# qianyizh/ElasticReconstruction

Measured on AMD Instinct MI355X. Metric: depth frames/sec into 512^3 TSDF (640x480), higher is better.
Workload: dtype f32; 1 GPU; configs[1]; frames_per_gpu=91800, volume_units_touched=122, warp=True, inputs=hbm_resident, parallelism=single GPU

## Files before the change

### elasticreconstruction_amd/_ffi.py

```python
import ctypes as C
import os

_HERE = os.path.dirname(os.path.abspath(__file__))
LIB_PATH = os.environ.get("ER_HIP_LIB") or os.path.join(_HERE, "liber_hip.so")

SYMBOLS = [
    "er_last_error", "er_device_count", "er_abi_version", "er_request_hw_queues", "er_host_alloc", "er_host_free", "er_host_copy_h2d", "er_device_alloc", "er_device_free", "er_device_copy_d2h",
    "er_tsdf_create", "er_tsdf_destroy", "er_tsdf_set_stream", "er_tsdf_synchronize",
    "er_tsdf_wait_event", "er_tsdf_reset", "er_tsdf_status", "er_tsdf_set_unit_shard", "er_unit_owner",
    "er_tsdf_scale_depth", "er_tsdf_reproject", "er_tsdf_integrate", "er_tsdf_integrate_frames",
    "er_tsdf_unit_count", "er_tsdf_unit_keys", "er_tsdf_read_unit", "er_tsdf_sum_weight",
    "er_tsdf_extract_world", "er_tsdf_extract_surface", "er_tsdf_extract_oriented", "er_tsdf_extract_mesh", "er_mc_table", "er_tsdf_extract_mesh_indexed", "er_tsdf_import_world", "er_raycast_params_default", "er_tsdf_raycast", "er_tsdf_raycast_batch", "er_tsdf_export_weighted", "er_tsdf_import_weighted",
    "er_tsdf_export_raw", "er_tsdf_import_raw",
    "er_tsdf_color_enable", "er_tsdf_read_unit_color", "er_tsdf_write_unit_color", "er_tsdf_color_frames", "er_tsdf_reproject_color", "er_tsdf_sample_colors",
    "er_tsdf_band_sizes", "er_tsdf_export_band", "er_tsdf_merge_band", "er_tsdf_import_band", "er_tsdf_drop_units",
    "er_tsdf_set_profiling", "er_tsdf_get_profile",
    "er_comm_unique_id", "er_comm_create", "er_comm_create_local", "er_comm_create_loopback", "er_comm_destroy", "er_comm_rank", "er_comm_world",
    "er_tsdf_allreduce", "er_comm_merge_stats", "er_comm_merge_stats_owner", "er_frame_block",
    "er_cloud_create", "er_cloud_create_batch", "er_cloud_create_from_tsdf", "er_cloud_destroy", "er_cloud_size",
    "er_icp_count_inliers", "er_icp_align", "er_icp_align_trace", "er_find_correspondence",
    "er_icp_count_inliers_batch", "er_icp_align_batch", "er_find_correspondence_batch", "er_icp_release_workspaces", "er_registration_batch", "er_ransac_fitness_batch", "er_ransac_inliers",
    "er_features_create", "er_features_destroy", "er_features_size", "er_feature_knn", "er_ransac_hypotheses", "er_ransac_params_default", "er_ransac_align", "er_ransac_align_batch",
    "er_odom_params_default", "er_odom_create", "er_odom_destroy", "er_odom_align_pairs", "er_odom_track", "er_frame_to_model_align", "er_frames_to_models_align", "er_odom_linearize", "er_odom_read_maps", "er_odom_tables",
    "er_cloud_read", "er_cloud_voxel_grid", "er_cloud_estimate_normals", "er_fpfh_estimate", "er_features_dim", "er_features_read",
    "er_frag_params_default", "er_frag_create", "er_frag_destroy", "er_frag_lane_bytes", "er_frag_build", "er_frag_count", "er_frag_read",
    "er_pgo_create", "er_pgo_destroy", "er_pgo_optimize", "er_pgo_set_state", "er_pgo_get_state", "er_pgo_linearize", "er_pgo_trial", "er_pgo_set_profiling", "er_pgo_get_profile",
    "er_fopt_create", "er_fopt_destroy", "er_fopt_set_cloud", "er_fopt_cloud_size", "er_fopt_get_points", "er_fopt_update_pose",
    "er_fopt_update_point_pn", "er_fopt_set_correspondences", "er_fopt_set_correspondences_dev", "er_fopt_group_count", "er_fopt_group_info", "er_fopt_update_normals", "er_fopt_assemble_rigid", "er_fopt_assemble_slac",
    "er_fopt_assemble_nonrigid", "er_fopt_factor_slac", "er_fopt_factor_nonrigid", "er_fopt_solve", "er_fopt_debug_shift_diagonal",
]


class ErWarp(C.Structure):
    _fields_ = [
        ("ctr", C.POINTER(C.c_float)),
        ("num_grids", C.c_int),
        ("resolution", C.c_int),
        ("length", C.c_float),
        ("grid_index", C.POINTER(C.c_int)),
        ("seg", C.POINTER(C.c_double)),
        ("madj", C.POINTER(C.c_double)),
    ]

# ... 34 lines not shown
        return _lib
    if not os.path.exists(LIB_PATH):
        raise ErError(
            "liber_hip.so not found at %s -- build it with `python -c 'import __graft_entry__ as g; g.build()'` "
            "or `make -C elasticreconstruction_amd/csrc`; there is no CPU fallback." % LIB_PATH)
    L = C.CDLL(LIB_PATH, mode=C.RTLD_GLOBAL)
    vp, ip, dp, fp = C.c_void_p, C.POINTER(C.c_int), C.POINTER(C.c_double), C.POINTER(C.c_float)
    u16p = C.POINTER(C.c_uint16)
    L.er_last_error.restype = C.c_char_p
    L.er_last_error.argtypes = []
    L.er_device_count.argtypes = []
    L.er_abi_version.argtypes = []
    L.er_host_alloc.restype = vp
    L.er_host_alloc.argtypes = [C.c_size_t]
    L.er_host_free.argtypes = [vp]
    L.er_host_copy_h2d.argtypes = [vp, vp, C.c_size_t]
    L.er_device_alloc.restype = vp
    L.er_device_alloc.argtypes = [C.c_size_t, C.c_int]
    L.er_device_free.argtypes = [vp]
    L.er_device_copy_d2h.argtypes = [vp, vp, C.c_size_t]
    L.er_tsdf_create.argtypes = [C.c_int, C.c_int, fp, C.c_int, C.c_int, C.POINTER(vp)]
    L.er_tsdf_destroy.argtypes = [vp]
    L.er_tsdf_set_stream.argtypes = [vp, vp]
    L.er_tsdf_synchronize.argtypes = [vp]
    L.er_tsdf_wait_event.argtypes = [vp, vp]
    L.er_tsdf_reset.argtypes = [vp]
    L.er_tsdf_status.argtypes = [vp, ip, C.POINTER(C.c_long)]
    L.er_tsdf_set_unit_shard.argtypes = [vp, C.c_int, C.c_int]
    L.er_unit_owner.argtypes = [C.c_int, C.c_int]
    L.er_tsdf_scale_depth.argtypes = [vp, vp, vp]
    L.er_tsdf_reproject.argtypes = [vp, vp, vp, C.c_int, C.c_float, vp, vp]
    L.er_tsdf_integrate.argtypes = [vp, vp, vp]
    L.er_tsdf_integrate_frames.argtypes = [vp, C.c_int, vp, C.c_int, vp, C.POINTER(ErWarp)]
    L.er_tsdf_unit_count.argtypes = [vp, ip]
    L.er_tsdf_unit_keys.argtypes = [vp, vp]
    L.er_tsdf_read_unit.argtypes = [vp, C.c_int, vp, vp]
    L.er_tsdf_sum_weight.argtypes = [vp, dp]
    L.er_tsdf_extract_world.argtypes = [vp, vp, C.c_long, C.POINTER(C.c_long)]
    L.er_tsdf_extract_surface.argtypes = [vp, vp, C.c_long, C.POINTER(C.c_long)]
    if hasattr(L, "er_tsdf_extract_oriented"):
        L.er_tsdf_extract_oriented.argtypes = [vp, vp, vp, C.c_long, C.POINTER(C.c_long)]
    L.er_tsdf_extract_mesh.argtypes = [vp, vp, C.c_long, C.POINTER(C.c_long)]
    L.er_mc_table.argtypes = [vp]
    if hasattr(L, "er_tsdf_extract_mesh_indexed"):
        L.er_tsdf_extract_mesh_indexed.argtypes = [vp, vp, vp, C.c_long, vp, C.c_long, C.POINTER(C.c_long), C.POINTER(C.c_long)]
        L.er_tsdf_import_world.argtypes = [vp, vp, C.c_long, ip]
    if hasattr(L, "er_tsdf_raycast"):
        L.er_raycast_params_default.argtypes = [C.POINTER(ErRaycastParams)]
        L.er_tsdf_raycast.argtypes = [vp, C.c_int, C.c_int, vp, vp, C.POINTER(ErRaycastParams), vp, vp, C.c_int]
    if hasattr(L, "er_tsdf_raycast_batch"):
        L.er_tsdf_raycast_batch.argtypes = [C.c_int, vp, vp, vp, vp, vp, vp, vp, vp]
    if hasattr(L, "er_frag_create"):
        L.er_frag_params_default.argtypes = [C.POINTER(ErFragParams)]
        L.er_frag_create.argtypes = [C.c_int, C.c_int, vp, C.POINTER(ErOdomParams), C.POINTER(ErFragParams), C.c_int, C.POINTER(vp)]
        L.er_frag_destroy.argtypes = [vp]
        L.er_frag_lane_bytes.argtypes = [vp, C.POINTER(C.c_size_t)]
        L.er_frag_build.argtypes = [vp, C.c_int, vp, C.c_int, vp, C.c_int, vp, vp]
        L.er_frag_count.argtypes = [vp, ip]
        L.er_frag_read.argtypes = [vp, C.c_int, vp, vp, C.c_long, C.POINTER(C.c_long)]
    if hasattr(L, "er_tsdf_color_enable"):
        L.er_tsdf_color_enable.argtypes = [vp]
        L.er_tsdf_read_unit_color.argtypes = [vp, C.c_int, vp]
        L.er_tsdf_write_unit_color.argtypes = [vp, C.c_int, vp]
        L.er_tsdf_color_frames.argtypes = [vp, C.c_int, vp, vp, C.c_int, vp, C.POINTER(ErWarp), vp]
        L.er_tsdf_sample_colors.argtypes = [vp, vp, C.c_long, vp, vp]
        L.er_tsdf_reproject_color.argtypes = [vp, vp, vp, vp, C.c_int, C.c_float, vp, vp]
# ... 158 lines not shown
```

### elasticreconstruction_amd/csrc/er_tsdf.h

```cpp
#pragma once

#include "er_common.h"
#include "er_tsdf_math.h"

#include "../../include/er_hip.h"

#include <algorithm>
#include <cstdlib>
#include <utility>
#include <vector>

namespace er_tsdf_k {
using namespace er;

constexpr int kBlock = 256;
constexpr int kEmptyKey = -1;
constexpr uint32_t kZEmpty = 0xFFFFFFFFu;

enum { C_NUNITS = 0, C_NBATCH = 1 , C_POOL_OVERFLOW = 2, C_TABLE_FULL = 3, C_OUT_OF_RANGE = 4,
       C_NBATCH1 = 6, C_NBATCH2 = 7, C_ZERO_WRITE = 8 ,
       C_ZERO_WRITE1 = 10, C_COUNT = 12 };
constexpr int kDepth = 3;
constexpr int kAux = 2;

struct ReprojArgs {
  const uint16_t* depth;
  int n_frames, cols, rows;
  Camera cam;
  CameraInv cami;
  const double* seg12;
  const double* madj12;
  const int* grid_index;
  const float* ctr;
  int res;
  float grid_ul;
  int floats_per_grid;
  uint32_t* zbuf;
  uint32_t* lastzero;
  uint32_t* zfix;
  int* zero_flag;
};
__global__ void k_reproject_scatter(ReprojArgs A);

constexpr int kFixThreads = 64;
constexpr int kFixBlocks = 256;

constexpr int kScaledPad = 64;
constexpr int kTile = 32;
constexpr int kLoShift = 4;
constexpr int kLoSub = kTile >> kLoShift;
constexpr int kTileKeys = 96;

constexpr int kPrepThreads = 256;
constexpr int kPrepPix = kTile * kTile / kPrepThreads;

__global__ __launch_bounds__(kPrepThreads) void k_prepare(
    const uint16_t* __restrict__ depth, uint32_t* __restrict__ zbuf, int n_frames, int cols, int rows,
    Camera cam, CameraInv cami, const float* __restrict__ lambda, const double* __restrict__ T12, float* __restrict__ scaled,
    int* __restrict__ ht_key, int* __restrict__ ht_slot, unsigned long long* __restrict__ ht_mask, int cap_mask,
    int hash_shift, int* __restrict__ batch, int* __restrict__ nbatch,
    int* __restrict__ counters, float* __restrict__ tile_max, float* __restrict__ tile_lo, float* __restrict__ tile_lo_fine, int2 shard,
    uint32_t* __restrict__ lastzero, uint32_t* __restrict__ zfix, const int* __restrict__ zero_flag);

constexpr int kRows = 4;
constexpr int kItemsPerUnit = 256;

struct Plan {
  int n_units;
  int next;
};

struct PlanRec {
  int key;
  int slot;
  unsigned long long mask;
};

constexpr int kIntMinBlocks = 5;

template <bool kSure>
__global__ __launch_bounds__(kBlock, kIntMinBlocks) void k_integrate(
    float2* __restrict__ pool, const PlanRec* __restrict__ plan_rec, Plan* __restrict__ plan,
    const FrameXform* __restrict__ frames, const float* __restrict__ scaled, const float* __restrict__ tile_max,
    const float* __restrict__ tile_lo, const float* __restrict__ tile_lo_fine, int tiles_x, int tiles_y, Camera cam, int cols, int rows);
extern template __global__ void k_integrate<true>(float2* __restrict__, const PlanRec* __restrict__, Plan* __restrict__, const FrameXform* __restrict__, const float* __restrict__, const float* __restrict__, const float* __restrict__, const float* __restrict__, int, int, Camera, int, int);
extern template __global__ void k_integrate<false>(float2* __restrict__, const PlanRec* __restrict__, Plan* __restrict__, const FrameXform* __restrict__, const float* __restrict__, const float* __restrict__, const float* __restrict__, const float* __restrict__, int, int, Camera, int, int);
}

struct er_tsdf_s {
  int device = 0, cols = 0, rows = 0, pixels = 0, max_units = 0;
  er::Camera cam{};
  er::CameraInv cami{};
  hipStream_t own_stream = nullptr, stream = nullptr;
  hipEvent_t caller_ev = nullptr;
  hipEvent_t voxel_done = nullptr;
// ... 57 lines not shown
```

### elasticreconstruction_amd/csrc/er_tsdf.hip

```cpp
#include "er_tsdf_dev.h"

namespace {

using namespace er_tsdf_k;

constexpr int kNbatchSlot[3] = {C_NBATCH, C_NBATCH1, C_NBATCH2};
constexpr int kZeroFlagSlot[2] = {C_ZERO_WRITE, C_ZERO_WRITE1};

__global__ void k_lambda(float* __restrict__ lambda, int cols, int rows, Camera cam) {
  int p = blockIdx.x * blockDim.x + threadIdx.x;
  if (p >= cols * rows) return;
  lambda[p] = scale_lambda(p % cols, p / cols, cam);
}

__global__ void k_scale_depth(const uint16_t* __restrict__ depth, const float* __restrict__ lambda,
                              float* __restrict__ scaled, int pixels, float itrunc) {
  int p = blockIdx.x * blockDim.x + threadIdx.x;
  if (p >= pixels) return;
  scaled[p] = scale_depth_px(depth[p], lambda[p], itrunc);
}

__global__ __launch_bounds__(kFixThreads) __attribute__((amdgpu_num_vgpr(48))) void k_reproject_fix(ReprojArgs A) {
  const int fl0 = A.zero_flag[0], fl1 = A.zero_flag[1];
  if ((fl0 | fl1) == 0) return;
// ... 296 lines not shown
  const double* dev_seg = reinterpret_cast<const double*>(dst + offsetof(Staging, seg));
  const double* dev_madj = reinterpret_cast<const double*>(dst + offsetof(Staging, madj));
  const int* dev_gi = reinterpret_cast<const int*>(dst + offsetof(Staging, gi));
  if (warp) {
    for (int f = 0; f < n; f++) {
      for (int q = 0; q < 12; q++) {
        st->seg[f * 16 + q] = warp->seg[(size_t)(frame0 + f) * 16 + q];
        st->madj[f * 12 + q] = warp->madj[(size_t)(frame0 + f) * 16 + q];
      }
      er::cube_coord_deltas(&st->seg[f * 16], h->cam, h->cols, h->rows, &st->seg[f * 16 + 12]);
      st->seg[f * 16 + 15] = 0.0;
      const int g = warp->grid_index[frame0 + f];
      if (g < 0 || g >= warp->num_grids) return er::fail("frame %d: control grid index %d out of [0,%d)", frame0 + f, g, warp->num_grids);
      st->gi[f] = g;
    }
  }
  if (h->used[p]) ER_HIP_TRY(hipStreamWaitEvent(X, h->int_done[p], 0));
  if (h->reset_pending[p]) {
    hipLaunchKernelGGL(k_reset, dim3(1), dim3(kBlock), 0, X, h->batch[p], nbatch, h->ht_mask[p], h->stats);
    ER_HIP_TRY(hipGetLastError());
    h->reset_pending[p] = false;
  }
  ER_HIP_TRY(hipMemcpyAsync(h->dstage[p], st, sizeof(Staging), hipMemcpyHostToDevice, X));
  ER_HIP_TRY(hipEventRecord(h->consts_done[p], X));
  if (warp) {
    const int verts = (warp->resolution + 1) * (warp->resolution + 1) * (warp->resolution + 1);
    const float grid_ul = warp->length / (float)warp->resolution;
    const ReprojArgs RA{depth_dev, n, h->cols, h->rows, h->cam, h->cami, dev_seg, dev_madj, dev_gi, h->ctr, warp->resolution, grid_ul,
                        verts * 3, h->zbuf[a], h->lastzero[a], h->zfix[a], h->counters + kZeroFlagSlot[a]};
    if (launch_reproject(h, RA, n, X)) return 1;
    zsrc = h->zbuf[a];
  }

  hipLaunchKernelGGL(k_prepare, dim3((h->cols + kTile - 1) / kTile, (h->rows + kTile - 1) / kTile, n), dim3(kPrepThreads), 0, X,
                     depth_dev, zsrc, n, h->cols, h->rows, h->cam, h->cami, h->lambda, dev_t12, h->scaled[p], h->ht_key, h->ht_slot,
                     h->ht_mask[p], h->ht_cap - 1, h->ht_shift, h->batch[p], nbatch, h->counters,
                     h->tile_max[p], h->tile_lo[p], h->tile_lo_fine[p], make_int2(h->shard_rank, h->shard_world), h->lastzero[a], h->zfix[a],
                     h->counters + kZeroFlagSlot[a]);
  hipLaunchKernelGGL(k_plan, dim3(1), dim3(256), 0, X, h->batch[p], nbatch, h->ht_mask[p], h->ht_key, h->ht_slot, h->unit_key, h->max_units,
                     h->counters, h->plan_rec[p], h->plan[p], warp ? h->counters + kZeroFlagSlot[a] : (int*)nullptr);
  ER_HIP_TRY(hipGetLastError());
  ER_HIP_TRY(hipEventRecord(h->pre_done[p], X));

  ER_HIP_TRY(hipStreamWaitEvent(S, h->pre_done[p], 0));
  hipEvent_t e0 = nullptr, e1 = nullptr;
  const bool timed = h->prof_stride > 0 && (h->prof_tick++ % h->prof_stride) == 0;
  if (timed) {
    ER_HIP_TRY(hipEventCreate(&e0));
    ER_HIP_TRY(hipEventCreate(&e1));
    ER_HIP_TRY(hipEventRecord(e0, S));
  }
  const bool sure = h->cam.integration_trunc < 64.0f;
  hipLaunchKernelGGL(sure ? k_integrate<true> : k_integrate<false>, dim3(wide_grid), dim3(kBlock), 0, S, h->pool, h->plan_rec[p], h->plan[p],
                     h->frames[p], h->scaled[p], h->tile_max[p], h->tile_lo[p], h->tile_lo_fine[p], (h->cols + kTile - 1) / kTile, (h->rows + kTile - 1) / kTile,
                     h->cam, h->cols, h->rows);
  if (timed) {
    ER_HIP_TRY(hipEventRecord(e1, S));
    h->events.emplace_back(e0, e1);
  }
  ER_HIP_TRY(hipGetLastError());
  ER_HIP_TRY(hipEventRecord(h->int_done[p], S));
  h->reset_pending[p] = true;
  h->used[p] = true;
  h->frames_done += n;
  return 0;
}

// ... 302 lines not shown
  for (int start = 0; start < n; start += per) {
    const int nb = std::min(per, n - start);
    const uint16_t* ddev;
    if (depth_on_device) {
      ddev = depth + (size_t)start * px;
    } else {
      const int p = (int)(h->batch_no % kDepth);
      if (!h->copy_stream) ER_HIP_TRY(hipStreamCreateWithFlags(&h->copy_stream, hipStreamNonBlocking));
      if (h->used[p]) ER_HIP_TRY(hipStreamWaitEvent(h->copy_stream, h->pre_done[p], 0));
      ER_HIP_TRY(hipMemcpyAsync(h->depth_stage[p], depth + (size_t)start * px, (size_t)nb * px * sizeof(uint16_t),
                                hipMemcpyHostToDevice, h->copy_stream));
      ER_HIP_TRY(hipEventRecord(h->copy_done[p], h->copy_stream));
      ER_HIP_TRY(hipStreamWaitEvent(h->aux_stream[h->batch_no % kAux], h->copy_done[p], 0));
      ddev = h->depth_stage[p];
    }
    if (run_batch(h, nb, ddev, T + (size_t)start * 16, warp, start)) return 1;
  }
  if (joined) {
    ER_HIP_TRY(hipEventRecord(h->voxel_done, h->own_stream));
    h->voxel_ahead = true;
  }
  if (warp) {
    for (int a = 0; a < kAux; a++) ER_HIP_TRY(hipEventRecord(h->ctr_rd[h->ctr_cur][a], h->aux_stream[a]));
    h->ctr_rd_set[h->ctr_cur] = true;
  }
  if (!depth_on_device && n > 0) ER_HIP_TRY(hipStreamSynchronize(h->copy_stream));
  return 0;
}

int er_tsdf_integrate(er_tsdf_t h, const uint16_t* depth_host, const double T[16]) {
  return er_tsdf_integrate_frames(h, 1, depth_host, 0, T, nullptr);
}

int er_tsdf_wait_event(er_tsdf_t h, void* hip_event) {
  if (!h || !hip_event) return er::fail("er_tsdf_wait_event: NULL argument");
  ER_HIP_TRY(hipSetDevice(h->device));
  for (int a = 0; a < kAux; a++) ER_HIP_TRY(hipStreamWaitEvent(h->aux_stream[a], (hipEvent_t)hip_event, 0));
  if (h->copy_stream) ER_HIP_TRY(hipStreamWaitEvent(h->copy_stream, (hipEvent_t)hip_event, 0));
  return 0;
}

int er_tsdf_reset(er_tsdf_t h) {
  if (!h) return er::fail("er_tsdf_reset: NULL handle");
  ER_HIP_TRY(hipSetDevice(h->device));
  if (sync_all(h)) return 1;
  int n = 0;
  ER_HIP_TRY(hipMemcpy(&n, h->counters + C_NUNITS, sizeof(int), hipMemcpyDeviceToHost));
  n = std::min(std::max(n, 0), h->max_units);
  hipStream_t s = h->stream;
  if (n > 0) ER_HIP_TRY(hipMemsetAsync(h->pool, 0, (size_t)n * er::kUnitVox * sizeof(float2), s));
  if (n > 0 && h->color) ER_HIP_TRY(hipMemsetAsync(h->color, 0, (size_t)n * er::kUnitVox * 16, s));
  ER_HIP_TRY(hipMemsetAsync(h->ht_key, 0xFF, (size_t)h->ht_cap * sizeof(int), s));
  ER_HIP_TRY(hipMemsetAsync(h->ht_slot, 0xFF, (size_t)h->ht_cap * sizeof(int), s));
  for (int q = 0; q < kDepth; q++) ER_HIP_TRY(hipMemsetAsync(h->ht_mask[q], 0, (size_t)h->ht_cap * sizeof(unsigned long long), s));
  ER_HIP_TRY(hipMemsetAsync(h->counters, 0, C_COUNT * sizeof(int), s));
  ER_HIP_TRY(hipStreamSynchronize(s));
  for (int q = 0; q < kDepth; q++) h->used[q] = h->reset_pending[q] = false;
  h->batch_no = 0;
  h->dropped.clear();
  return 0;
}

int er_tsdf_set_unit_shard(er_tsdf_t h, int rank, int world) {
  if (!h) return er::fail("er_tsdf_set_unit_shard: NULL handle");
  if (world < 1 || rank < 0 || rank >= world) return er::fail("er_tsdf_set_unit_shard: rank %d not in [0,%d)", rank, world);
  ER_HIP_TRY(hipSetDevice(h->device));
// ... 121 lines not shown
```

### elasticreconstruction_amd/csrc/er_tsdf_pre.hip

```cpp
#include "er_tsdf_dev.h"

namespace er_tsdf_k {

__global__ void k_reproject_scatter(ReprojArgs A) {
  const int f = blockIdx.z;
  const int u = blockIdx.x * 64 + (threadIdx.x & 63);
  const int v = blockIdx.y * 4 + (threadIdx.x >> 6);
  if (u >= A.cols || v >= A.rows) return;
  reproject_scatter_px(A, f, u, v, 0);
}

namespace {

__device__ void touch_unit(int key, int f, int* __restrict__ ht_key, int* __restrict__ ht_slot,
                           unsigned long long* __restrict__ ht_mask, int cap_mask, int hash_shift,
                           int* __restrict__ batch, int* __restrict__ nbatch, int* __restrict__ counters, int2 shard) {
  if (shard.y > 1 && unit_owner(key, shard.y) != shard.x) return;
  const int e = ht_find_or_insert(ht_key, cap_mask, hash_shift, key);
  if (e < 0) {
    atomicOr(&counters[C_TABLE_FULL], 1);
    return;
  }
  const unsigned long long bit = 1ull << f;
  const unsigned long long seen = __hip_atomic_load(&ht_mask[e], __ATOMIC_RELAXED, __HIP_MEMORY_SCOPE_AGENT);
  if (seen & bit) return;
  const unsigned long long old = atomicOr(&ht_mask[e], bit);
  if (old != 0ull) return;
  batch[atomicAdd(nbatch, 1)] = e;
}

}

__global__ __launch_bounds__(kPrepThreads) void k_prepare(
    const uint16_t* __restrict__ depth, uint32_t* __restrict__ zbuf, int n_frames, int cols, int rows,
    Camera cam, CameraInv cami, const float* __restrict__ lambda, const double* __restrict__ T12, float* __restrict__ scaled,
    int* __restrict__ ht_key, int* __restrict__ ht_slot, unsigned long long* __restrict__ ht_mask, int cap_mask,
    int hash_shift, int* __restrict__ batch, int* __restrict__ nbatch,
    int* __restrict__ counters, float* __restrict__ tile_max, float* __restrict__ tile_lo, float* __restrict__ tile_lo_fine, int2 shard,
    uint32_t* __restrict__ lastzero, uint32_t* __restrict__ zfix, const int* __restrict__ zero_flag) {
  __shared__ int s_keys[kTileKeys];
  __shared__ int s_n;
  __shared__ float s_wmax[kPrepThreads / 64], s_wlo[kLoSub][kLoSub][kPrepThreads / 64];
  const int pixels = cols * rows;
  const int f = blockIdx.z;
  const bool replayed = zbuf && ((zero_flag[f >> 5] >> (f & 31)) & 1);
  const int tx = threadIdx.x & (kTile - 1), ty = threadIdx.x >> 5;
  const int x = blockIdx.x * kTile + tx;
  if (threadIdx.x == 0) s_n = 0;
  __syncthreads();
  uint16_t d[kPrepPix];
  float lam[kPrepPix];
#pragma unroll
  for (int q = 0; q < kPrepPix; q++) {
    const int y = blockIdx.y * kTile + ty + q * (kTile / kPrepPix);
    d[q] = 0;
    lam[q] = 0.0f;
    if (x < cols && y < rows) {
      const int p = y * cols + x;
      const size_t o = (size_t)f * pixels + p;
      if (zbuf) {
        uint32_t z = zbuf[o];
        zbuf[o] = kZEmpty;
        if (replayed) z = take_z(z, o, lastzero, zfix);
        d[q] = (z == kZEmpty) ? (uint16_t)0 : (uint16_t)z;
      } else {
        d[q] = depth[o];
      }
      lam[q] = lambda[p];
    }
  }
  float wmax = 0.0f, vlo[kPrepPix];
#pragma unroll
  for (int q = 0; q < kPrepPix; q++) vlo[q] = 3.0e38f;
#pragma unroll
  for (int q = 0; q < kPrepPix; q++) {
    const int y = blockIdx.y * kTile + ty + q * (kTile / kPrepPix);
    int key = -1;
    if (x < cols && y < rows) {
      const float sc = scale_depth_px(d[q], lam[q], cam.integration_trunc);
      scaled[(size_t)f * (pixels + kScaledPad) + y * cols + x] = sc;
      wmax = fmaxf(wmax, sc);
      vlo[q] = sc > 0.001f ? sc : 0.0f;
      if (d[q] > 0) {
        key = touch_key(x, y, d[q], cam, cami, T12 + f * 12);
        if (key < 0) atomicAdd(&counters[C_OUT_OF_RANGE], 1);
      }
    }
    const int left = __shfl_up(key, 1);
    const bool leader = key >= 0 && (tx == 0 || left != key);
    if (leader) {
      const int slot = atomicAdd(&s_n, 1);
      if (slot < kTileKeys) {
        s_keys[slot] = key;
      } else {
        touch_unit(key, f, ht_key, ht_slot, ht_mask, cap_mask, hash_shift, batch, nbatch, counters, shard);
      }
    }
  }
  for (int off = 32; off > 0; off >>= 1) wmax = fmaxf(wmax, __shfl_xor(wmax, off));
  if ((threadIdx.x & 63) == 0) s_wmax[threadIdx.x >> 6] = wmax;
  {
    constexpr int qper = kPrepPix / kLoSub;
#pragma unroll
    for (int sr = 0; sr < kLoSub; sr++) {
      float r = vlo[sr * qper];
#pragma unroll
      for (int e = 1; e < qper; e++) r = fminf(r, vlo[sr * qper + e]);
#pragma unroll
      for (int off = 1; off < (1 << kLoShift); off <<= 1) r = fminf(r, __shfl_xor(r, off));
      r = fminf(r, __shfl_xor(r, 32));
      if ((threadIdx.x & 32) == 0 && (tx & ((1 << kLoShift) - 1)) == 0) s_wlo[sr][tx >> kLoShift][threadIdx.x >> 6] = r;
    }
  }
  __syncthreads();
  if (threadIdx.x == 0) {
    float m = 0.0f, lo = 3.0e38f;
    for (int w = 0; w < kPrepThreads / 64; w++) m = fmaxf(m, s_wmax[w]);
    for (int e = 0; e < kLoSub * kLoSub * (kPrepThreads / 64); e++) lo = fminf(lo, (&s_wlo[0][0][0])[e]);
    const size_t t = ((size_t)blockIdx.y * gridDim.x + blockIdx.x) * ER_MAX_BATCH + f;
    tile_max[t] = m;
    tile_lo[t] = lo;
  }
  if ((int)threadIdx.x < kLoSub * kLoSub) {
    const int sr = threadIdx.x / kLoSub, sg = threadIdx.x % kLoSub;
    float lo = 3.0e38f;
    for (int w = 0; w < kPrepThreads / 64; w++) lo = fminf(lo, s_wlo[sr][sg][w]);
    const int lx = blockIdx.x * kLoSub + sg, ly = blockIdx.y * kLoSub + sr;
    const int lo_tx = (cols + (1 << kLoShift) - 1) >> kLoShift, lo_ty = (rows + (1 << kLoShift) - 1) >> kLoShift;
    if (lx < lo_tx && ly < lo_ty) tile_lo_fine[((size_t)ly * lo_tx + lx) * ER_MAX_BATCH + f] = lo;
  }
  const int n = min(s_n, kTileKeys);
  if ((int)threadIdx.x < n) {
    const int k = s_keys[threadIdx.x];
    bool dup = false;
    for (int j = 0; j < (int)threadIdx.x; j++) dup = dup || (s_keys[j] == k);
    if (!dup) touch_unit(k, f, ht_key, ht_slot, ht_mask, cap_mask, hash_shift, batch, nbatch, counters, shard);
  }
}

}
```

### elasticreconstruction_amd/tsdf.py

```python
import ctypes as C
import os

import numpy as np

from . import _ffi
from . import formats

UNIT_VOX = 64 * 64 * 64


def mat4_mul(A, B):
    A = np.asarray(A, np.float64)
    B = np.asarray(B, np.float64)
    out = np.empty((4, 4), np.float64)
    for r in range(4):
        for c in range(4):
            out[r, c] = ((A[r, 0] * B[0, c] + A[r, 1] * B[1, c]) + A[r, 2] * B[2, c]) + A[r, 3] * B[3, c]
    return out


class TSDFVolume:

    def __init__(self, cols=640, rows=480, camera=None, max_units=1024, device=0):
        self._lib = _ffi.lib()
# ... 60 lines not shown
        d = np.ascontiguousarray(depth, dtype=np.uint16).reshape(-1)
        T = np.ascontiguousarray(transformation, dtype=np.float64).reshape(16)
        _ffi.check(self._lib.er_tsdf_integrate(self._h, _ffi.ptr(d), _ffi.ptr(T)), "er_tsdf_integrate")

    @staticmethod
    def _warp_ref(warp, n):
        if warp is None:
            return None, []
        ctr = np.ascontiguousarray(warp["ctr"], dtype=np.float32)
        gi = np.ascontiguousarray(warp["grid_index"], dtype=np.int32).reshape(-1)
        seg = np.ascontiguousarray(warp["seg"], dtype=np.float64).reshape(-1, 16)
        madj = np.ascontiguousarray(warp["madj"], dtype=np.float64).reshape(-1, 16)
        assert gi.size == n and seg.shape[0] == n and madj.shape[0] == n
        res = int(warp["resolution"])
        num = ctr.size // (3 * (res + 1) ** 3)
        w = _ffi.ErWarp(ctr.ctypes.data_as(C.POINTER(C.c_float)), num, res, C.c_float(warp["length"]),
                        gi.ctypes.data_as(C.POINTER(C.c_int)), seg.ctypes.data_as(C.POINTER(C.c_double)),
                        madj.ctypes.data_as(C.POINTER(C.c_double)))
        return C.byref(w), [ctr, gi, seg, madj, w]

    def IntegrateFrames(self, depth, transformations, warp=None, device_ptr=None):
        T = np.ascontiguousarray(transformations, dtype=np.float64).reshape(-1, 16)
        n = T.shape[0]
        w_ref, keep = self._warp_ref(warp, n)
        if device_ptr is not None:
            _ffi.check(self._lib.er_tsdf_integrate_frames(self._h, n, C.c_void_p(device_ptr), 1, _ffi.ptr(T), w_ref),
                       "er_tsdf_integrate_frames")
        else:
            d = np.ascontiguousarray(depth, dtype=np.uint16).reshape(n, -1)
            assert d.shape[1] == self.cols_ * self.rows_
            _ffi.check(self._lib.er_tsdf_integrate_frames(self._h, n, _ffi.ptr(d), 0, _ffi.ptr(T), w_ref),
                       "er_tsdf_integrate_frames")
        del keep

    def unit_count(self):
        n = C.c_int(0)
        _ffi.check(self._lib.er_tsdf_unit_count(self._h, C.byref(n)), "er_tsdf_unit_count")
        return n.value

    def unit_keys(self):
        n = self.unit_count()
        keys = np.empty(n, dtype=np.int32)
        if n:
            _ffi.check(self._lib.er_tsdf_unit_keys(self._h, _ffi.ptr(keys)), "er_tsdf_unit_keys")
        return keys

    def read_unit(self, key):
        sdf = np.empty(UNIT_VOX, dtype=np.float32)
        w = np.empty(UNIT_VOX, dtype=np.float32)
        _ffi.check(self._lib.er_tsdf_read_unit(self._h, int(key), _ffi.ptr(sdf), _ffi.ptr(w)), "er_tsdf_read_unit")
        return sdf, w

    def sum_weight(self):
        s = C.c_double(0)
        _ffi.check(self._lib.er_tsdf_sum_weight(self._h, C.byref(s)), "er_tsdf_sum_weight")
        return s.value

    def extract_world(self):
        n = C.c_long(0)
        _ffi.check(self._lib.er_tsdf_extract_world(self._h, None, 0, C.byref(n)), "er_tsdf_extract_world")
        out = np.empty((n.value, 4), dtype=np.float32)
        if n.value:
            _ffi.check(self._lib.er_tsdf_extract_world(self._h, _ffi.ptr(out), n.value, C.byref(n)), "er_tsdf_extract_world")
        return out

    def extract_surface(self):
# ... 370 lines not shown
```

### include/er_hip.h

```cpp
#ifndef ER_HIP_H_
#define ER_HIP_H_

#include <stddef.h>
#include <stdint.h>

#ifdef __cplusplus
extern "C" {
#endif

#define ER_UNIT_RES 64
#define ER_UNIT_VOX (64 * 64 * 64)
#define ER_MAX_BATCH 64

const char* er_last_error(void);
int er_device_count(void);
int er_abi_version(void);
int er_request_hw_queues(int n);

void* er_host_alloc(size_t bytes);
int er_host_free(void* p);
int er_host_copy_h2d(void* dev_dst, const void* host_src, size_t bytes);
void* er_device_alloc(size_t bytes, int device);
int er_device_free(void* p);
int er_device_copy_d2h(void* host_dst, const void* dev_src, size_t bytes);

typedef struct er_tsdf_s* er_tsdf_t;

typedef struct er_warp {
  const float* ctr;
  int num_grids;
  int resolution;
  float length;
  const int* grid_index;
  const double* seg;
  const double* madj;
} er_warp;

int er_tsdf_create(int cols, int rows, const float cam6[6], int max_units, int device, er_tsdf_t* out);
int er_tsdf_destroy(er_tsdf_t h);

int er_tsdf_set_stream(er_tsdf_t h, void* hip_stream);
int er_tsdf_synchronize(er_tsdf_t h);

int er_tsdf_scale_depth(er_tsdf_t h, const uint16_t* depth_host, float* scaled_host);

int er_tsdf_reproject(er_tsdf_t h, uint16_t* depth_inout_host, const float* ctr_host, int resolution, float length,
                      const double seg[16], const double madj[16]);

int er_tsdf_integrate(er_tsdf_t h, const uint16_t* depth_host, const double T[16]);

int er_tsdf_integrate_frames(er_tsdf_t h, int n, const uint16_t* depth, int depth_on_device, const double* T,
                             const er_warp* warp);

int er_tsdf_wait_event(er_tsdf_t h, void* hip_event);

int er_tsdf_reset(er_tsdf_t h);

#define ER_STATUS_POOL_EXHAUSTED 1
#define ER_STATUS_TABLE_FULL 2
int er_tsdf_status(er_tsdf_t h, int* flags, long* out_of_range_pixels);

int er_tsdf_unit_count(er_tsdf_t h, int* count);
int er_tsdf_unit_keys(er_tsdf_t h, int* keys_host);
int er_tsdf_read_unit(er_tsdf_t h, int key, float* sdf_host, float* weight_host);

int er_tsdf_sum_weight(er_tsdf_t h, double* sum);

int er_tsdf_extract_world(er_tsdf_t h, float* out_host, long capacity, long* count);

int er_tsdf_extract_surface(er_tsdf_t h, float* out_host, long capacity, long* count);

int er_tsdf_extract_oriented(er_tsdf_t h, float* points_host, float* normals_host, long capacity, long* count);

int er_tsdf_extract_mesh(er_tsdf_t h, float* tri_host, long capacity_triangles, long* n_triangles);
int er_mc_table(unsigned char out[256 * 16]);

int er_tsdf_extract_mesh_indexed(er_tsdf_t h, float* verts_host, float* normals_host, long capacity_vertices, int* tri_host,
                                 long capacity_triangles, long* n_vertices, long* n_triangles);

int er_tsdf_import_world(er_tsdf_t h, const float* xyzi_host, long n, int* n_units);

int er_tsdf_color_enable(er_tsdf_t h);

int er_tsdf_read_unit_color(er_tsdf_t h, int key, uint32_t* rgbn_host);
int er_tsdf_write_unit_color(er_tsdf_t h, int key, const uint32_t* rgbn_host);
// ... 258 lines not shown
```

Baseline: 188,500 frames/s.

## Vectorize k_prepare to four horizontal pixels per thread with DPP reductions

Reworks the depth prepare kernel so each thread handles four adjacent pixels in a row instead of four rows of one column. This allows 8/16-byte vector loads of depth, zbuf and lambda and a vector store of the scaled depth. The warp shuffles for max/min tile reductions and the neighbour key check are replaced with DPP and permlane swaps. A templated wide path is selected when alignment allows, with a scalar fallback. A trace entry point is added for validating prepass outputs.

```diff
diff --git a/elasticreconstruction_amd/_ffi.py b/elasticreconstruction_amd/_ffi.py
--- a/elasticreconstruction_amd/_ffi.py
+++ b/elasticreconstruction_amd/_ffi.py
@@ -8,7 +8,7 @@
     "er_last_error", "er_device_count", "er_abi_version", "er_request_hw_queues", "er_host_alloc", "er_host_free", "er_host_copy_h2d", "er_device_alloc", "er_device_free", "er_device_copy_d2h",
     "er_tsdf_create", "er_tsdf_destroy", "er_tsdf_set_stream", "er_tsdf_synchronize",
     "er_tsdf_wait_event", "er_tsdf_reset", "er_tsdf_status", "er_tsdf_set_unit_shard", "er_unit_owner",
-    "er_tsdf_scale_depth", "er_tsdf_reproject", "er_tsdf_integrate", "er_tsdf_integrate_frames",
+    "er_tsdf_scale_depth", "er_tsdf_reproject", "er_tsdf_integrate", "er_tsdf_integrate_frames", "er_tsdf_prepass_trace",
     "er_tsdf_unit_count", "er_tsdf_unit_keys", "er_tsdf_read_unit", "er_tsdf_sum_weight",
     "er_tsdf_extract_world", "er_tsdf_extract_surface", "er_tsdf_extract_oriented", "er_tsdf_extract_mesh", "er_mc_table", "er_tsdf_extract_mesh_indexed", "er_tsdf_import_world", "er_raycast_params_default", "er_tsdf_raycast", "er_tsdf_raycast_batch", "er_tsdf_export_weighted", "er_tsdf_import_weighted",
     "er_tsdf_export_raw", "er_tsdf_import_raw",
@@ -109,6 +109,8 @@
     L.er_tsdf_reproject.argtypes = [vp, vp, vp, C.c_int, C.c_float, vp, vp]
     L.er_tsdf_integrate.argtypes = [vp, vp, vp]
     L.er_tsdf_integrate_frames.argtypes = [vp, C.c_int, vp, C.c_int, vp, C.POINTER(ErWarp)]
+    if hasattr(L, "er_tsdf_prepass_trace"):
+        L.er_tsdf_prepass_trace.argtypes = [vp, C.c_int, vp, C.c_int, vp, C.POINTER(ErWarp), vp, ip, vp, vp, vp, vp, vp, C.c_int, ip]
     L.er_tsdf_unit_count.argtypes = [vp, ip]
     L.er_tsdf_unit_keys.argtypes = [vp, vp]
     L.er_tsdf_read_unit.argtypes = [vp, C.c_int, vp, vp]
diff --git a/elasticreconstruction_amd/csrc/er_tsdf.h b/elasticreconstruction_amd/csrc/er_tsdf.h
--- a/elasticreconstruction_amd/csrc/er_tsdf.h
+++ b/elasticreconstruction_amd/csrc/er_tsdf.h
@@ -54,6 +54,7 @@
 constexpr int kPrepThreads = 256;
 constexpr int kPrepPix = kTile * kTile / kPrepThreads;
 
+template <bool kWide>
 __global__ __launch_bounds__(kPrepThreads) void k_prepare(
     const uint16_t* __restrict__ depth, uint32_t* __restrict__ zbuf, int n_frames, int cols, int rows,
     Camera cam, CameraInv cami, const float* __restrict__ lambda, const double* __restrict__ T12, float* __restrict__ scaled,
@@ -61,6 +62,8 @@
     int hash_shift, int* __restrict__ batch, int* __restrict__ nbatch,
     int* __restrict__ counters, float* __restrict__ tile_max, float* __restrict__ tile_lo, float* __restrict__ tile_lo_fine, int2 shard,
     uint32_t* __restrict__ lastzero, uint32_t* __restrict__ zfix, const int* __restrict__ zero_flag);
+extern template __global__ void k_prepare<true>(const uint16_t* __restrict__, uint32_t* __restrict__, int, int, int, Camera, CameraInv, const float* __restrict__, const double* __restrict__, float* __restrict__, int* __restrict__, int* __restrict__, unsigned long long* __restrict__, int, int, int* __restrict__, int* __restrict__, int* __restrict__, float* __restrict__, float* __restrict__, float* __restrict__, int2, uint32_t* __restrict__, uint32_t* __restrict__, const int* __restrict__);
+extern template __global__ void k_prepare<false>(const uint16_t* __restrict__, uint32_t* __restrict__, int, int, int, Camera, CameraInv, const float* __restrict__, const double* __restrict__, float* __restrict__, int* __restrict__, int* __restrict__, unsigned long long* __restrict__, int, int, int* __restrict__, int* __restrict__, int* __restrict__, float* __restrict__, float* __restrict__, float* __restrict__, int2, uint32_t* __restrict__, uint32_t* __restrict__, const int* __restrict__);
 
 constexpr int kRows = 4;
 constexpr int kItemsPerUnit = 256;
diff --git a/elasticreconstruction_amd/csrc/er_tsdf.hip b/elasticreconstruction_amd/csrc/er_tsdf.hip
--- a/elasticreconstruction_amd/csrc/er_tsdf.hip
+++ b/elasticreconstruction_amd/csrc/er_tsdf.hip
@@ -352,7 +352,8 @@
     zsrc = h->zbuf[a];
   }
 
-  hipLaunchKernelGGL(k_prepare, dim3((h->cols + kTile - 1) / kTile, (h->rows + kTile - 1) / kTile, n), dim3(kPrepThreads), 0, X,
+  const bool wide = h->cols % 4 == 0 && (zsrc || reinterpret_cast<uintptr_t>(depth_dev) % 8 == 0);
+  hipLaunchKernelGGL(wide ? k_prepare<true> : k_prepare<false>, dim3((h->cols + kTile - 1) / kTile, (h->rows + kTile - 1) / kTile, n), dim3(kPrepThreads), 0, X,
                      depth_dev, zsrc, n, h->cols, h->rows, h->cam, h->cami, h->lambda, dev_t12, h->scaled[p], h->ht_key, h->ht_slot,
                      h->ht_mask[p], h->ht_cap - 1, h->ht_shift, h->batch[p], nbatch, h->counters,
                      h->tile_max[p], h->tile_lo[p], h->tile_lo_fine[p], make_int2(h->shard_rank, h->shard_world), h->lastzero[a], h->zfix[a],
@@ -721,6 +722,40 @@
   return er_tsdf_integrate_frames(h, 1, depth_host, 0, T, nullptr);
 }
 
+int er_tsdf_prepass_trace(er_tsdf_t h, int n, const uint16_t* depth, int depth_on_device, const double* T, const er_warp* warp,
+                          float* scaled, int* scaled_pad, float* tile_max, float* tile_lo, float* tile_lo_fine,
+                          int* keys, unsigned long long* masks, int keys_cap, int* n_keys) {
+  if (!h) return er::fail("er_tsdf_prepass_trace: NULL handle");
+  if (n < 1 || n > ER_MAX_BATCH) return er::fail("er_tsdf_prepass_trace: %d frames outside 1..%d (one batch)", n, ER_MAX_BATCH);
+  ER_HIP_TRY(hipSetDevice(h->device));
+  if (sync_all(h)) return 1;
+  const int p = (int)(h->batch_no % kDepth);
+  if (er_tsdf_integrate_frames(h, n, depth, depth_on_device, T, warp)) return 1;
+  if (sync_all(h)) return 1;
+  const size_t B = ER_MAX_BATCH, px = (size_t)h->pixels;
+  const size_t tiles = (size_t)((h->cols + kTile - 1) / kTile) * ((h->rows + kTile - 1) / kTile);
+  const size_t fine = (size_t)((h->cols + (1 << kLoShift) - 1) >> kLoShift) * ((h->rows + (1 << kLoShift) - 1) >> kLoShift);
+  if (scaled_pad) *scaled_pad = kScaledPad;
+  if (scaled) ER_HIP_TRY(hipMemcpy(scaled, h->scaled[p], (size_t)n * (px + kScaledPad) * sizeof(float), hipMemcpyDeviceToHost));
+  if (tile_max) ER_HIP_TRY(hipMemcpy(tile_max, h->tile_max[p], tiles * B * sizeof(float), hipMemcpyDeviceToHost));
+  if (tile_lo) ER_HIP_TRY(hipMemcpy(tile_lo, h->tile_lo[p], tiles * B * sizeof(float), hipMemcpyDeviceToHost));
+  if (tile_lo_fine) ER_HIP_TRY(hipMemcpy(tile_lo_fine, h->tile_lo_fine[p], fine * B * sizeof(float), hipMemcpyDeviceToHost));
+  Plan plan{};
+  ER_HIP_TRY(hipMemcpy(&plan, h->plan[p], sizeof plan, hipMemcpyDeviceToHost));
+  if (plan.n_units < 0 || plan.n_units > h->ht_cap) return er::fail("er_tsdf_prepass_trace: the batch lists %d units", plan.n_units);
+  if (n_keys) *n_keys = plan.n_units;
+  if (keys || masks) {
+    std::vector<PlanRec> rec((size_t)plan.n_units);
+    if (plan.n_units > 0) ER_HIP_TRY(hipMemcpy(rec.data(), h->plan_rec[p], rec.size() * sizeof(PlanRec), hipMemcpyDeviceToHost));
+    std::sort(rec.begin(), rec.end(), [](const PlanRec& a, const PlanRec& b) { return a.key < b.key; });
+    for (int i = 0; i < plan.n_units && i < keys_cap; i++) {
+      if (keys) keys[i] = rec[(size_t)i].key;
+      if (masks) masks[i] = rec[(size_t)i].mask;
+    }
+  }
+  return 0;
+}
+
 int er_tsdf_wait_event(er_tsdf_t h, void* hip_event) {
   if (!h || !hip_event) return er::fail("er_tsdf_wait_event: NULL argument");
   ER_HIP_TRY(hipSetDevice(h->device));
diff --git a/elasticreconstruction_amd/csrc/er_tsdf_pre.hip b/elasticreconstruction_amd/csrc/er_tsdf_pre.hip
--- a/elasticreconstruction_amd/csrc/er_tsdf_pre.hip
+++ b/elasticreconstruction_amd/csrc/er_tsdf_pre.hip
@@ -31,6 +31,62 @@
 
 }
 
+namespace {
+
+template <int kCtrl>
+__device__ __forceinline__ int dpp_mov(int v) {
+  return __builtin_amdgcn_update_dpp(v, v, kCtrl, 0xF, 0xF, false);
+}
+constexpr int kDppQuadXor1 = 0xB1;
+constexpr int kDppQuadXor2 = 0x4E;
+constexpr int kDppRowShr1 = 0x111;
+constexpr int kDppRowRor4 = 0x124;
+constexpr int kDppRowRor8 = 0x128;
+
+template <int kCtrl>
+__device__ __forceinline__ float dpp_movf(float v) {
+  return __int_as_float(dpp_mov<kCtrl>(__float_as_int(v)));
+}
+
+struct FMin { __device__ __forceinline__ float operator()(float a, float b) const { return fminf(a, b); } };
+struct FMax { __device__ __forceinline__ float operator()(float a, float b) const { return fmaxf(a, b); } };
+
+template <class Op>
+__device__ __forceinline__ float across_rows(float v, Op op) {
+  const unsigned u = (unsigned)__float_as_int(v);
+  const auto s16 = __builtin_amdgcn_permlane16_swap(u, u, false, false);
+  v = op(__int_as_float((int)s16[0]), __int_as_float((int)s16[1]));
+  const unsigned w = (unsigned)__float_as_int(v);
+  const auto s32 = __builtin_amdgcn_permlane32_swap(w, w, false, false);
+  return op(__int_as_float((int)s32[0]), __int_as_float((int)s32[1]));
+}
+
+template <class Op>
+__device__ __forceinline__ float reduce_half_columns(float v, Op op) {
+  v = op(v, dpp_movf<kDppQuadXor1>(v));
+  v = op(v, dpp_movf<kDppQuadXor2>(v));
+  v = op(v, dpp_movf<kDppRowRor8>(v));
+  return across_rows(v, op);
+}
+
+template <class Op>
+__device__ __forceinline__ float reduce_wave(float v, Op op) {
+  v = op(v, dpp_movf<kDppQuadXor1>(v));
+  v = op(v, dpp_movf<kDppQuadXor2>(v));
+  v = op(v, dpp_movf<kDppRowRor4>(v));
+  v = op(v, dpp_movf<kDppRowRor8>(v));
+  return across_rows(v, op);
+}
+
+}
+
+static_assert(kTile == 32 && kPrepPix == 4 && kPrepThreads == 256, "k_prepare: 8 column groups x 32 rows of 4 pixels; a wave is 8 rows of the tile");
+static_assert(kLoShift == 4 && kLoSub == 2, "k_prepare: a sub-tile is 4 threads (one quad) wide and 2 waves high; lane bit 2 is its column");
+constexpr int kPrepCols = kTile / kPrepPix;
+constexpr int kPrepWaveRows = 64 / kPrepCols;
+constexpr int kPrepSubWaves = (1 << kLoShift) / kPrepWaveRows;
+
+template <bool kWide>
 __global__ __launch_bounds__(kPrepThreads) void k_prepare(
     const uint16_t* __restrict__ depth, uint32_t* __restrict__ zbuf, int n_frames, int cols, int rows,
     Camera cam, CameraInv cami, const float* __restrict__ lambda, const double* __restrict__ T12, float* __restrict__ scaled,
@@ -40,83 +96,111 @@
     uint32_t* __restrict__ lastzero, uint32_t* __restrict__ zfix, const int* __restrict__ zero_flag) {
   __shared__ int s_keys[kTileKeys];
   __shared__ int s_n;
-  __shared__ float s_wmax[kPrepThreads / 64], s_wlo[kLoSub][kLoSub][kPrepThreads / 64];
+  __shared__ float s_wmax[kPrepThreads / 64], s_wlo[kLoSub][kLoSub][kPrepSubWaves];
   const int pixels = cols * rows;
   const int f = blockIdx.z;
   const bool replayed = zbuf && ((zero_flag[f >> 5] >> (f & 31)) & 1);
-  const int tx = threadIdx.x & (kTile - 1), ty = threadIdx.x >> 5;
-  const int x = blockIdx.x * kTile + tx;
+  const int c = threadIdx.x & (kPrepCols - 1), r = threadIdx.x / kPrepCols;
+  const int x0 = blockIdx.x * kTile + c * kPrepPix, y = blockIdx.y * kTile + r;
   if (threadIdx.x == 0) s_n = 0;
   __syncthreads();
+  const int p = y * cols + x0;
+  const size_t o = (size_t)f * pixels + p;
+  float* __restrict__ const sc_out = scaled + ((size_t)f * (pixels + kScaledPad) + p);
   uint16_t d[kPrepPix];
   float lam[kPrepPix];
-#pragma unroll
-  for (int q = 0; q < kPrepPix; q++) {
-    const int y = blockIdx.y * kTile + ty + q * (kTile / kPrepPix);
-    d[q] = 0;
-    lam[q] = 0.0f;
-    if (x < cols && y < rows) {
-      const int p = y * cols + x;
-      const size_t o = (size_t)f * pixels + p;
+  bool in[kPrepPix];
+#pragma unroll
+  for (int j = 0; j < kPrepPix; j++) {
+    d[j] = 0;
+    lam[j] = 0.0f;
+    in[j] = y < rows && x0 + (kWide ? 0 : j) < cols;
+  }
+  if constexpr (kWide) {
+    if (in[0]) {
       if (zbuf) {
-        uint32_t z = zbuf[o];
-        zbuf[o] = kZEmpty;
-        if (replayed) z = take_z(z, o, lastzero, zfix);
-        d[q] = (z == kZEmpty) ? (uint16_t)0 : (uint16_t)z;
+        const uint4 zv = *reinterpret_cast<const uint4*>(zbuf + o);
+        *reinterpret_cast<uint4*>(zbuf + o) = make_uint4(kZEmpty, kZEmpty, kZEmpty, kZEmpty);
+        uint32_t z[kPrepPix] = {zv.x, zv.y, zv.z, zv.w};
+        if (replayed) {
+#pragma unroll
+          for (int j = 0; j < kPrepPix; j++) z[j] = take_z(z[j], o + j, lastzero, zfix);
+        }
+#pragma unroll
+        for (int j = 0; j < kPrepPix; j++) d[j] = (z[j] == kZEmpty) ? (uint16_t)0 : (uint16_t)z[j];
       } else {
-        d[q] = depth[o];
-      }
-      lam[q] = lambda[p];
-    }
-  }
-  float wmax = 0.0f, vlo[kPrepPix];
-#pragma unroll
-  for (int q = 0; q < kPrepPix; q++) vlo[q] = 3.0e38f;
-#pragma unroll
-  for (int q = 0; q < kPrepPix; q++) {
-    const int y = blockIdx.y * kTile + ty + q * (kTile / kPrepPix);
-    int key = -1;
-    if (x < cols && y < rows) {
-      const float sc = scale_depth_px(d[q], lam[q], cam.integration_trunc);
-      scaled[(size_t)f * (pixels + kScaledPad) + y * cols + x] = sc;
-      wmax = fmaxf(wmax, sc);
-      vlo[q] = sc > 0.001f ? sc : 0.0f;
-      if (d[q] > 0) {
-        key = touch_key(x, y, d[q], cam, cami, T12 + f * 12);
-        if (key < 0) atomicAdd(&counters[C_OUT_OF_RANGE], 1);
-      }
-    }
-    const int left = __shfl_up(key, 1);
-    const bool leader = key >= 0 && (tx == 0 || left != key);
+        uint2 dv;
+        __builtin_memcpy(&dv, __builtin_assume_aligned(depth + o, 8), 8);
+        d[0] = (uint16_t)dv.x;
+        d[1] = (uint16_t)(dv.x >> 16);
+        d[2] = (uint16_t)dv.y;
+        d[3] = (uint16_t)(dv.y >> 16);
+      }
+      const float4 lv = *reinterpret_cast<const float4*>(lambda + p);
+      lam[0] = lv.x;
+      lam[1] = lv.y;
+      lam[2] = lv.z;
+      lam[3] = lv.w;
+    }
+  } else {
+#pragma unroll
+    for (int j = 0; j < kPrepPix; j++) {
+      if (in[j]) {
+        if (zbuf) {
+          uint32_t z = zbuf[o + j];
+          zbuf[o + j] = kZEmpty;
+          if (replayed) z = take_z(z, o + j, lastzero, zfix);
+          d[j] = (z == kZEmpty) ? (uint16_t)0 : (uint16_t)z;
+        } else {
+          d[j] = depth[o + j];
+        }
+        lam[j] = lambda[p + j];
+      }
+    }
+  }
+  float wmax = 0.0f, vlo = 3.0e38f, sc[kPrepPix];
+  int key[kPrepPix];
+#pragma unroll
+  for (int j = 0; j < kPrepPix; j++) {
+    key[j] = -1;
+    sc[j] = 0.0f;
+    if (in[j]) {
+      sc[j] = scale_depth_px(d[j], lam[j], cam.integration_trunc);
+      if constexpr (!kWide) sc_out[j] = sc[j];
+      wmax = fmaxf(wmax, sc[j]);
+      vlo = fminf(vlo, sc[j] > 0.001f ? sc[j] : 0.0f);
+      if (d[j] > 0) {
+        key[j] = touch_key(x0 + j, y, d[j], cam, cami, T12 + f * 12);
+        if (key[j] < 0) atomicAdd(&counters[C_OUT_OF_RANGE], 1);
+      }
+    }
+  }
+  if constexpr (kWide) {
+    if (in[0]) *reinterpret_cast<float4*>(sc_out) = make_float4(sc[0], sc[1], sc[2], sc[3]);
+  }
+  const int left = dpp_mov<kDppRowShr1>(key[kPrepPix - 1]);
+#pragma unroll
+  for (int j = 0; j < kPrepPix; j++) {
+    const bool leader = key[j] >= 0 && (j == 0 ? (c == 0 || left != key[0]) : key[j - 1] != key[j]);
     if (leader) {
       const int slot = atomicAdd(&s_n, 1);
       if (slot < kTileKeys) {
-        s_keys[slot] = key;
+        s_keys[slot] = key[j];
       } else {
-        touch_unit(key, f, ht_key, ht_slot, ht_mask, cap_mask, hash_shift, batch, nbatch, counters, shard);
-      }
-    }
-  }
-  for (int off = 32; off > 0; off >>= 1) wmax = fmaxf(wmax, __shfl_xor(wmax, off));
-  if ((threadIdx.x & 63) == 0) s_wmax[threadIdx.x >> 6] = wmax;
-  {
-    constexpr int qper = kPrepPix / kLoSub;
-#pragma unroll
-    for (int sr = 0; sr < kLoSub; sr++) {
-      float r = vlo[sr * qper];
-#pragma unroll
-      for (int e = 1; e < qper; e++) r = fminf(r, vlo[sr * qper + e]);
-#pragma unroll
-      for (int off = 1; off < (1 << kLoShift); off <<= 1) r = fminf(r, __shfl_xor(r, off));
-      r = fminf(r, __shfl_xor(r, 32));
-      if ((threadIdx.x & 32) == 0 && (tx & ((1 << kLoShift) - 1)) == 0) s_wlo[sr][tx >> kLoShift][threadIdx.x >> 6] = r;
-    }
-  }
+        touch_unit(key[j], f, ht_key, ht_slot, ht_mask, cap_mask, hash_shift, batch, nbatch, counters, shard);
+      }
+    }
+  }
+  const int lane = threadIdx.x & 63, wave = threadIdx.x >> 6;
+  wmax = reduce_wave(wmax, FMax());
+  vlo = reduce_half_columns(vlo, FMin());
+  if (lane == 0) s_wmax[wave] = wmax;
+  if ((lane & ~4) == 0) s_wlo[wave / kPrepSubWaves][lane >> 2][wave % kPrepSubWaves] = vlo;
   __syncthreads();
   if (threadIdx.x == 0) {
     float m = 0.0f, lo = 3.0e38f;
     for (int w = 0; w < kPrepThreads / 64; w++) m = fmaxf(m, s_wmax[w]);
-    for (int e = 0; e < kLoSub * kLoSub * (kPrepThreads / 64); e++) lo = fminf(lo, (&s_wlo[0][0][0])[e]);
+    for (int e = 0; e < kLoSub * kLoSub * kPrepSubWaves; e++) lo = fminf(lo, (&s_wlo[0][0][0])[e]);
     const size_t t = ((size_t)blockIdx.y * gridDim.x + blockIdx.x) * ER_MAX_BATCH + f;
     tile_max[t] = m;
     tile_lo[t] = lo;
@@ -124,7 +208,7 @@
   if ((int)threadIdx.x < kLoSub * kLoSub) {
     const int sr = threadIdx.x / kLoSub, sg = threadIdx.x % kLoSub;
     float lo = 3.0e38f;
-    for (int w = 0; w < kPrepThreads / 64; w++) lo = fminf(lo, s_wlo[sr][sg][w]);
+    for (int w = 0; w < kPrepSubWaves; w++) lo = fminf(lo, s_wlo[sr][sg][w]);
     const int lx = blockIdx.x * kLoSub + sg, ly = blockIdx.y * kLoSub + sr;
     const int lo_tx = (cols + (1 << kLoShift) - 1) >> kLoShift, lo_ty = (rows + (1 << kLoShift) - 1) >> kLoShift;
     if (lx < lo_tx && ly < lo_ty) tile_lo_fine[((size_t)ly * lo_tx + lx) * ER_MAX_BATCH + f] = lo;
@@ -138,4 +222,14 @@
   }
 }
 
-}
+#define ER_PREPARE_INST(W) \
+  template __global__ void k_prepare<W>(const uint16_t* __restrict__, uint32_t* __restrict__, int, int, int, Camera, CameraInv, const float* __restrict__, \
+                                        const double* __restrict__, float* __restrict__, int* __restrict__, int* __restrict__,                             \
+                                        unsigned long long* __restrict__, int, int, int* __restrict__, int* __restrict__, int* __restrict__,               \
+                                        float* __restrict__, float* __restrict__, float* __restrict__, int2, uint32_t* __restrict__,                       \
+                                        uint32_t* __restrict__, const int* __restrict__);
+ER_PREPARE_INST(true)
+ER_PREPARE_INST(false)
+#undef ER_PREPARE_INST
+
+}
diff --git a/elasticreconstruction_amd/tsdf.py b/elasticreconstruction_amd/tsdf.py
--- a/elasticreconstruction_amd/tsdf.py
+++ b/elasticreconstruction_amd/tsdf.py
@@ -116,6 +116,35 @@
             _ffi.check(self._lib.er_tsdf_integrate_frames(self._h, n, _ffi.ptr(d), 0, _ffi.ptr(T), w_ref),
                        "er_tsdf_integrate_frames")
         del keep
+
+    def prepass_trace(self, depth, transformations, warp=None, device_ptr=None):
+        T = np.ascontiguousarray(transformations, dtype=np.float64).reshape(-1, 16)
+        n = T.shape[0]
+        w_ref, keep = self._warp_ref(warp, n)
+        px = self.cols_ * self.rows_
+        if device_ptr is not None:
+            src, on_dev = C.c_void_p(device_ptr), 1
+        else:
+            d = np.ascontiguousarray(depth, dtype=np.uint16).reshape(n, -1)
+            assert d.shape[1] == px
+            src, on_dev = _ffi.ptr(d), 0
+        B = 64
+        tx, ty = (self.cols_ + 31) // 32, (self.rows_ + 31) // 32
+        fx, fy = (self.cols_ + 15) // 16, (self.rows_ + 15) // 16
+        pad, nk = C.c_int(0), C.c_int(0)
+        pad_floats = 64
+        scaled = np.empty((n, px + pad_floats), np.float32)
+        tmax, tlo = np.empty((ty, tx, B), np.float32), np.empty((ty, tx, B), np.float32)
+        fine = np.empty((fy, fx, B), np.float32)
+        cap = 1 << 16
+        keys, masks = np.empty(cap, np.int32), np.empty(cap, np.uint64)
+        _ffi.check(self._lib.er_tsdf_prepass_trace(self._h, n, src, on_dev, _ffi.ptr(T), w_ref, _ffi.ptr(scaled), C.byref(pad), _ffi.ptr(tmax),
+                                                   _ffi.ptr(tlo), _ffi.ptr(fine), _ffi.ptr(keys), _ffi.ptr(masks), cap, C.byref(nk)),
+                   "er_tsdf_prepass_trace")
+        del keep
+        assert pad.value == pad_floats and nk.value <= cap
+        return dict(scaled=scaled, pad=pad.value, tile_max=tmax[:, :, :n].copy(), tile_lo=tlo[:, :, :n].copy(),
+                    tile_lo_fine=fine[:, :, :n].copy(), keys=keys[:nk.value].copy(), masks=masks[:nk.value].copy())
 
     def unit_count(self):
         n = C.c_int(0)
diff --git a/include/er_hip.h b/include/er_hip.h
--- a/include/er_hip.h
+++ b/include/er_hip.h
@@ -51,6 +51,10 @@
 
 int er_tsdf_integrate_frames(er_tsdf_t h, int n, const uint16_t* depth, int depth_on_device, const double* T,
                              const er_warp* warp);
+
+int er_tsdf_prepass_trace(er_tsdf_t h, int n, const uint16_t* depth, int depth_on_device, const double* T, const er_warp* warp,
+                          float* scaled, int* scaled_pad, float* tile_max, float* tile_lo, float* tile_lo_fine,
+                          int* keys, unsigned long long* masks, int keys_cap, int* n_keys);
 
 int er_tsdf_wait_event(er_tsdf_t h, void* hip_event);
 
```

New measurement: 193,900 frames/s, median of 6. 2.9% higher.
